# chubbymaggie/syzkaller

Hardware: AMD Instinct MI355X
Metric: signal elems triaged/sec (Diff+Merge) (higher is better)
Workload: dtype u32

## Files before the change

syzkaller_amd/csrc/agg.hip:

```cpp
#include <algorithm>
#include <vector>

#include "decide.h"
#include "internal.h"

namespace syz {

constexpr uint32_t kAggThreads = 1024;
constexpr uint32_t kAggSlots = 7424;
constexpr uint32_t kAggBW = 4;
using KBucket = uint4;
constexpr uint32_t kAggBuckets = kAggSlots / kAggBW;
constexpr uint32_t kAggNoSlot = 0xFFFFFFFFu;
static_assert(kAggRegion == kAggSlots, "distinct-list region per partition (internal.h)");
constexpr uint32_t kAggLimit = kAggSlots * 4 / 5;
constexpr double kAggTargetLoad = 0.4;
constexpr double kAggTargetLoadEntry = 0.6;
constexpr uint64_t kMinItems = 2048;
constexpr uint32_t kAggEmpty = 0xFFFFFFFFu;
constexpr uint32_t kAggOverflow = 0xFFFFFFFFu;
constexpr uint32_t kAggMinBits = 3, kAggMaxBits = 11;
constexpr uint32_t kAggMaxParts = 1u << kAggMaxBits;
constexpr uint32_t kAggTile = 18432;
constexpr uint32_t kAggGroup = 8;
constexpr uint32_t kAggU = 4, kAggD = 2;

struct AggGeom {
	uint32_t pbits;
	uint32_t ibits;
	__host__ __device__ uint32_t rbits() const { return 32 - pbits; }
	__host__ __device__ uint32_t cbits() const { return pbits - 2; }
	__host__ __device__ uint32_t items_per_chunk_log2() const { return cbits() - ibits; }
	__host__ __device__ uint32_t part(uint32_t h) const { return h >> (32 - pbits); }
	__host__ __device__ uint32_t meta(uint32_t level, uint64_t serial) const
	{
		return (level << cbits()) | ((uint32_t)serial & ((1u << cbits()) - 1));
	}
	__host__ __device__ uint32_t rec(uint32_t h, uint32_t meta) const { return (h << pbits) | meta; }
	__host__ __device__ uint32_t resid(uint32_t r) const { return r >> pbits; }
	__host__ __device__ uint32_t level(uint32_t r) const { return (r >> cbits()) & 3; }
	__host__ __device__ uint32_t local(uint32_t r) const { return r & ((1u << cbits()) - 1); }
};

__device__ __forceinline__ uint32_t agg_home_bucket(uint32_t key, const AggGeom& g)
{
	return __umulhi(key << g.pbits, kAggBuckets);
}

__device__ __forceinline__ uint32_t lds_flag(uint32_t* f)
{
	return __hip_atomic_load(f, __ATOMIC_RELAXED, __HIP_MEMORY_SCOPE_WORKGROUP);
}
__device__ __forceinline__ void lds_flag_set(uint32_t* f)
{
	__hip_atomic_store(f, 1u, __ATOMIC_RELAXED, __HIP_MEMORY_SCOPE_WORKGROUP);
}

__device__ __forceinline__ uint32_t bucket_find(uint4 B, uint32_t e)
{
	return B.x == e ? 0 : B.y == e ? 1 : B.z == e ? 2 : B.w == e ? 3 : 4;
}

__device__ __forceinline__ uint32_t bucket_first_empty(uint4 B)
{
	return B.x == kAggEmpty ? 0 : B.y == kAggEmpty ? 1 : B.z == kAggEmpty ? 2 : B.w == kAggEmpty ? 3 : 4;
}

__device__ uint32_t agg_find_insert(KBucket* kb, uint32_t e, uint32_t b, KBucket B, uint32_t* s_ovf, uint32_t& ins)
{
	uint32_t* keys = reinterpret_cast<uint32_t*>(kb);
	for (uint32_t step = 0; step < kAggBuckets;) {
		const uint32_t f = bucket_find(B, e);
		if (f < kAggBW)
			return b * kAggBW + f;
		const uint32_t j = bucket_first_empty(B);
		if (j == kAggBW) {
			b = b + 1 == kAggBuckets ? 0 : b + 1;
			B = kb[b];
			step++;
			continue;
		}
		const uint32_t i = b * kAggBW + j;
		const uint32_t key = atomicCAS(&keys[i], kAggEmpty, e);
		if (key == kAggEmpty) {
			ins++;
			return i;
		}
		if (key == e)
			return i;
		B = kb[b];
	}
	lds_flag_set(s_ovf);
	return kAggNoSlot;
}

struct CellGroup {
	uint64_t ch0;
	uint32_t bnd[kAggGroup + 1];
	__device__ void load(const uint32_t* __restrict__ ot, uint64_t nchunks, uint64_t gi)
	{
		ch0 = gi * kAggGroup;
#pragma unroll
		for (uint32_t i = 0; i <= kAggGroup; i++)
			bnd[i] = ot[min<uint64_t>(ch0 + i, nchunks)];
	}
	__device__ uint32_t serial(uint32_t j, uint32_t r, const AggGeom& g) const
	{
		uint32_t chunk = (uint32_t)ch0;
#pragma unroll
		for (uint32_t i = 1; i < kAggGroup; i++)
			chunk += j >= bnd[i];
		return (chunk << g.cbits()) | g.local(r);
	}
};

template <bool kShard>
__global__ __launch_bounds__(kAggThreads) void k_agg_count(const uint32_t* __restrict__ sigs,
                                                           const uint64_t* __restrict__ call_start,
                                                           const uint32_t* __restrict__ call_len, uint64_t c0,
                                                           uint64_t c1, AggGeom g, AggSrc x, uint32_t* counts)
{
	__shared__ uint32_t h[kAggMaxParts];
	auto add = [&](uint32_t e) {
		if (!kShard || owner_of(e, x.nshards) == x.shard)
			atomicAdd(&h[g.part(fmix32(e))], 1u);
	};
	const uint32_t P = 1u << g.pbits, cb = g.ibits;
	const uint32_t w = threadIdx.x >> 6, nw = blockDim.x >> 6, lane = lane_id();
	const uint64_t ncalls = c1 - c0, nchunks = (ncalls + (1ull << cb) - 1) >> cb;
	for (uint64_t ch = blockIdx.x; ch < nchunks; ch += gridDim.x) {
		for (uint32_t i = threadIdx.x; i < P; i += blockDim.x)
			h[i] = 0;
		__syncthreads();
		const uint64_t ce = min<uint64_t>(ncalls, (ch + 1) << cb);
		for (uint64_t s = (ch << cb) + w; s < ce; s += nw) {
			const uint64_t c = c0 + s, start = call_start[c];
			const uint32_t len = call_len[c];
			uint32_t j = lane;
			for (; j + 192 < len; j += 256) {
				const uint32_t a = sigs[start + j], b = sigs[start + j + 64], d = sigs[start + j + 128],
				               f = sigs[start + j + 192];
				add(a);
				add(b);
				add(d);
				add(f);
			}
			for (; j < len; j += 64)
				add(sigs[start + j]);
		}
		__syncthreads();
		for (uint32_t i = threadIdx.x; i < P; i += blockDim.x)
			counts[ch * P + i] = h[i];
		__syncthreads();
	}
}

__device__ __forceinline__ uint32_t block_excl_scan_1k(uint32_t v, uint32_t* out)
{
	__shared__ uint32_t wsum[16];
	const uint32_t lane = lane_id(), w = threadIdx.x >> 6, nw = blockDim.x >> 6;
	uint32_t x = v;
#pragma unroll
	for (int o = 1; o < 64; o <<= 1) {
		const uint32_t y = __shfl_up(x, o, 64);
		if (lane >= (uint32_t)o)
			x += y;
	}
	if (lane == 63)
		wsum[w] = x;
	__syncthreads();
	uint32_t pre = 0, tot = 0;
	for (uint32_t i = 0; i < nw; i++) {
		pre += i < w ? wsum[i] : 0;
		tot += wsum[i];
	}
	__syncthreads();
	*out = pre + x - v;
	return tot;
}

__global__ __launch_bounds__(1024) void k_agg_scan_chunks(const uint32_t* counts, uint64_t nitems, uint32_t ilog,
                                                          uint32_t P, uint32_t* offs, uint32_t* offsT, uint64_t* totals)
{
	const uint32_t p = blockIdx.x;
	const uint64_t nchunks = (nitems + (1ull << ilog) - 1) >> ilog;
	uint32_t* ot = offsT + (uint64_t)p * (nchunks + 1);
	uint64_t run = 0;
	for (uint64_t b0 = 0; b0 < nitems; b0 += blockDim.x) {
		const uint64_t b = b0 + threadIdx.x;
		const uint32_t v = b < nitems ? counts[b * P + p] : 0;
		uint32_t ex;
		const uint32_t tot = block_excl_scan_1k(v, &ex);
		if (b < nitems) {
			offs[b * P + p] = (uint32_t)(run + ex);
			if ((b & ((1ull << ilog) - 1)) == 0)
				ot[b >> ilog] = (uint32_t)(run + ex);
		}
		run += tot;
	}
	if (threadIdx.x == 0) {
		totals[p] = run;
		ot[nchunks] = (uint32_t)run;
	}
}

__global__ __launch_bounds__(1024) void k_agg_scan_totals(const uint64_t* totals, uint32_t P, uint64_t* rec_base)
{
	__shared__ uint64_t wsum[16];
	const uint32_t lane = lane_id(), w = threadIdx.x >> 6, i0 = threadIdx.x * 2;
	const uint64_t a = i0 < P ? totals[i0] : 0, b = i0 + 1 < P ? totals[i0 + 1] : 0;
	uint64_t x = a + b;
#pragma unroll
	for (int o = 1; o < 64; o <<= 1) {
		const uint64_t y = __shfl_up(x, o, 64);
		if (lane >= (uint32_t)o)
			x += y;
	}
	if (lane == 63)
		wsum[w] = x;
	__syncthreads();
	uint64_t pre = 0, tot = 0;
	for (uint32_t k = 0; k < 16; k++) {
		pre += k < w ? wsum[k] : 0;
		tot += wsum[k];
	}
	const uint64_t ex = pre + x - (a + b);
	if (i0 < P)
		rec_base[i0] = ex;
	if (i0 + 1 < P)
		rec_base[i0 + 1] = ex + a;
	if (threadIdx.x == 0)
		rec_base[P] = tot;
}

constexpr uint32_t kScatChunkMax = 1u << (kAggMaxBits - 2);
constexpr uint32_t kScatWaves = kAggThreads / 64;

constexpr uint32_t kScat3K = 16;
constexpr uint32_t kScat3KEntry = 10;
constexpr uint32_t kScat3Fill = 85;
constexpr uint32_t kScatPer = 12;
constexpr uint32_t kScatPerEntry = 10;
constexpr uint32_t kBlk = 16;
constexpr uint32_t kDummyLines = 2048;
typedef uint32_t scat_v4u __attribute__((ext_vector_type(4)));

struct CapCells {
	const uint64_t* base;
	const uint32_t* cap;
	uint32_t* cnt;
	uint32_t* ovf;
	uint64_t nchunks;
	uint32_t* dummy;
	const uint64_t* sizes = nullptr;
	const uint32_t* tiles = nullptr;
	bool split = false;
	uint32_t tile = 1024;
};

constexpr uint32_t kScat3Tile = kScat3K * 64, kScat3TileEntry = kScat3KEntry * 64;
__host__ __device__ inline uint64_t scat3_tiles(uint32_t len, uint32_t tile)
{
	return (len + tile - 1) / tile;
}
__device__ inline bool scat3_takes(uint64_t recs, uint32_t tiles, uint32_t tile)
{
	return recs * 100 >= (uint64_t)tiles * tile * kScat3Fill;
}

template <bool kOn>
struct PrioLevels {
	uint8_t lvl[kOn ? 256 : 1];
	__device__ __forceinline__ void load(const LevelMap& lm, uint32_t nthreads)
	{
		if (kOn) {
			for (uint32_t i = threadIdx.x; i < 256; i += nthreads)
				lvl[i] = lm.lvl[i];
		}
	}
	__device__ __forceinline__ uint32_t level(uint32_t pv, bool kept, bool& bad) const
	{
		const uint32_t lv = lvl[kOn ? pv : 0];
		bad |= kept && lv == 0xff;
		return lv & 3;
	}
	static __device__ __forceinline__ void report(bool bad, const AggSrc& x)
	{
		if (kOn && x.bad_level && __ballot(bad) && lane_id() == 0)
			atomicOr(x.bad_level, 1u);
	}
};

struct CallTable {
	uint64_t start[kScatChunkMax];
	uint32_t len[kScatChunkMax];
	uint16_t meta[kScatChunkMax];
	template <bool kEntry>
	__device__ __forceinline__ void load(const uint64_t* __restrict__ call_start, const uint32_t* __restrict__ call_len,
	                                     const uint8_t* __restrict__ call_prio, const LevelMap& lm, const AggGeom& g,
	                                     uint64_t c0, uint64_t cbeg, uint32_t nc)
	{
		for (uint32_t i = threadIdx.x; i < nc; i += blockDim.x) {
			const uint64_t c = c0 + cbeg + i;
			start[i] = call_start[c];
			len[i] = call_len[c];
			meta[i] = (uint16_t)g.meta(kEntry ? 0 : lm.lvl[call_prio[c]], cbeg + i);
		}
	}
	__device__ __forceinline__ uint32_t call_of(uint32_t w, uint32_t loc) const { return w + (loc >> 24) * kScatWaves; }
	template <bool kEntry, uint32_t kPer>
	__device__ __forceinline__ uint32_t fetch(uint32_t w, uint32_t lane, uint32_t nc, uint32_t& wc, uint32_t& wo,
	                                          const uint32_t* __restrict__ sigs, const AggSrc& x, uint32_t (&ev)[kPer],
	                                          uint32_t (&loc)[kPer], uint32_t (&pv)[kEntry ? kPer : 1]) const
	{
		constexpr uint32_t kQuota = kPer * 64;
		uint32_t q = 0;
		while (q < kQuota && wc < nc) {
			const uint32_t ln = len[wc], m = min(kQuota - q, ln - wo);
			const uint32_t tag = ((wc - w) / kScatWaves) << 24;
			if (q == 0) {
#pragma unroll
				for (uint32_t u = 0; u < kPer; u++)
					loc[u] = tag | wo;
			}
#pragma unroll
			for (uint32_t u = 0; u < kPer; u++) {
				const uint32_t i = u * 64 + lane;
				loc[u] = i >= q && i < q + m ? tag | (wo + i - q) : loc[u];
			}
			q += m;
			wo += m;
			if (wo == ln) {
				wc += kScatWaves;
				wo = 0;
			}
		}
		if (q) {
#pragma unroll
			for (uint32_t u = 0; u < kPer; u++) {
				const uint64_t a = start[call_of(w, loc[u])] + (loc[u] & 0xFFFFFFu);
				ev[u] = __builtin_nontemporal_load(&sigs[a]);
				if (kEntry)
					pv[kEntry ? u : 0] = (uint8_t)__builtin_nontemporal_load(&x.elem_prio[a]);
			}
		}
		return q;
	}
};

template <bool kEntry>
__global__ __launch_bounds__(kAggThreads) void k_agg_scatter(const uint32_t* __restrict__ sigs,
                                                             const uint64_t* __restrict__ call_start,
                                                             const uint32_t* __restrict__ call_len,
                                                             const uint8_t* __restrict__ call_prio, LevelMap lm,
                                                             uint64_t c0, uint64_t c1, AggGeom g, AggSrc x,
                                                             const uint32_t* __restrict__ offs,
                                                             const uint64_t* __restrict__ rec_base, uint32_t* recs)
{
	constexpr uint32_t kQuota = kAggTile / kScatWaves, kPer = kQuota / 64;
	static_assert(kQuota % 64 == 0, "tile quota per wave");
	__shared__ uint32_t t_rec[kAggTile];
	__shared__ uint16_t t_part[kAggTile];
	__shared__ uint64_t cur[kAggMaxParts];
	__shared__ uint32_t hist[kAggMaxParts], pos[kAggMaxParts];
	__shared__ CallTable calls;
	__shared__ PrioLevels<kEntry> levels;
	const uint32_t P = 1u << g.pbits, cb = g.cbits(), ib = g.ibits;
	levels.load(lm, blockDim.x);
	const uint32_t w = threadIdx.x >> 6, lane = lane_id();
	const uint64_t ncalls = c1 - c0, nitems = (ncalls + (1ull << ib) - 1) >> ib;
	const uint32_t per_t = (P + blockDim.x - 1) / blockDim.x;
	bool badlv = false;
	for (uint64_t ch = blockIdx.x; ch < nitems; ch += gridDim.x) {
		const uint64_t cbeg = ch << ib;
		const uint32_t nc = (uint32_t)min<uint64_t>(ncalls - cbeg, 1ull << ib);
		for (uint32_t i = threadIdx.x; i < P; i += blockDim.x) {
			cur[i] = rec_base[i] + offs[ch * P + i];
			hist[i] = 0;
		}
		calls.load<kEntry>(call_start, call_len, call_prio, lm, g, c0, cbeg, nc);
		__syncthreads();
		uint32_t wc = w, wo = 0;
		uint32_t ev[kPer], loc[kPer], pv[kEntry ? kPer : 1];
		auto fetch = [&]() { return calls.fetch<kEntry>(w, lane, nc, wc, wo, sigs, x, ev, loc, pv); };
		uint32_t n = fetch();
		for (;;) {
#pragma unroll
			for (uint32_t u = 0; u < kPer; u++) {
				const uint32_t i = u * 64 + lane;
				const bool keep = i < n && (!kEntry || x.nshards == 1 || owner_of(ev[u], x.nshards) == x.shard);
				if (keep) {
					const uint32_t h = fmix32(ev[u]), p = g.part(h);
					const uint32_t r = atomicAdd(&hist[p], 1u);
					uint32_t meta = calls.meta[calls.call_of(w, loc[u])];
					if (kEntry)
						meta |= levels.level(pv[kEntry ? u : 0], true, badlv) << cb;
					ev[u] = g.rec(h, meta);
					loc[u] = p | (r << 16);
				} else {
					loc[u] = ~0u;
				}
			}
			__syncthreads();
			uint32_t hsum = 0;
			for (uint32_t q = 0; q < per_t; q++) {
				const uint32_t i = threadIdx.x * per_t + q;
				hsum += i < P ? hist[i] : 0;
			}
			uint32_t ex;
			const uint32_t nt = block_excl_scan_1k(hsum, &ex);
			for (uint32_t q = 0; q < per_t; q++) {
				const uint32_t i = threadIdx.x * per_t + q;
				if (i < P) {
					pos[i] = ex;
					cur[i] -= ex;
					ex += hist[i];
				}
			}
			__syncthreads();
#pragma unroll
			for (uint32_t u = 0; u < kPer; u++) {
				if (loc[u] != ~0u) {
					const uint32_t p = loc[u] & 0xFFFFu, d = pos[p] + (loc[u] >> 16);
					t_rec[d] = ev[u];
					t_part[d] = (uint16_t)p;
				}
			}
			n = fetch();
			__syncthreads();
			for (uint32_t d = threadIdx.x; d < nt; d += blockDim.x)
				recs[cur[t_part[d]] + d] = t_rec[d];
			__syncthreads();
			for (uint32_t i = threadIdx.x; i < P; i += blockDim.x) {
				cur[i] += pos[i] + hist[i];
				hist[i] = 0;
			}
			if (!__syncthreads_or(n != 0))
				break;
		}
	}
	PrioLevels<kEntry>::report(badlv, x);
}

struct ScatLane {
	uint32_t w, lane;
	uint32_t seq = 0;
	bool spilled = false;
};
struct ScatItem {
	uint32_t* recs;
	uint64_t base;
	uint32_t cap;
};
template <uint32_t kB>
struct ScatBlocks {
	static_assert(kB == 16 || kB == 32, "block of 64 or 128 B");
	static constexpr uint32_t kMaxP = kB == 16 ? 2048 : 1024;
	static_assert(kMaxP * kB * 4 == 128 * 1024 && kMaxP <= kAggMaxParts, "128 KB of blocks");
	static constexpr uint32_t kG = 64 / kB;
	static constexpr uint32_t kLB = kB / 4, kGF = 64 / kLB;
	static constexpr uint32_t kShare = (kMaxP + kAggThreads - 1) / kAggThreads;
	alignas(16) uint32_t buf[kMaxP * kB];
	uint32_t fillc[kMaxP + 1];
	uint32_t written[kMaxP + 1];
	uint16_t flist[kShare * kAggThreads];
	uint32_t s_or[2][kScatWaves];

	__device__ __forceinline__ void reset(uint32_t P)
	{
		for (uint32_t i = threadIdx.x; i < P; i += kAggThreads) {
			fillc[i] = 0;
			written[i] = 0;
		}
	}
	__device__ __forceinline__ bool wg_or(ScatLane& t, bool pred)
	{
		uint32_t* r = s_or[t.seq++ & 1];
		const bool any = __ballot(pred) != 0;
		if (t.lane == 0)
			r[t.w] = any;
		__syncthreads();
		return __ballot(r[t.lane & (kScatWaves - 1)] != 0) != 0;
	}
	template <uint32_t M>
	__device__ __forceinline__ uint32_t place(const uint32_t (&rec)[M], const uint32_t (&pt)[M], uint32_t pend)
	{
		uint32_t sl[M];
#pragma unroll
		for (uint32_t u = 0; u < M; u++)
			sl[u] = (pend >> u) & 1 ? atomicAdd(&fillc[pt[u]], 1u) : kB;
#pragma unroll
		for (uint32_t u = 0; u < M; u++) {
			if (sl[u] < kB) {
				buf[pt[u] * kB + sl[u]] = rec[u];
				pend &= ~(1u << u);
			}
		}
		return pend;
	}
	__device__ __forceinline__ void flush(ScatLane& t, uint32_t P, const ScatItem& it, uint32_t* dummy)
	{
		const uint32_t fgrp = t.lane / kLB, fq = t.lane % kLB;
		uint16_t* wl = flist + t.w * kShare * 64;
		uint32_t nw = 0;
#pragma unroll
		for (uint32_t i = 0; i < kShare; i++) {
			const uint32_t p = i * kAggThreads + t.w * 64 + t.lane;
			const bool f = p < P && fillc[p] >= kB;
			const uint64_t m = __ballot(f);
			if (f)
				wl[nw + lane_rank(m)] = (uint16_t)p;
			nw += (uint32_t)__popcll(m);
		}
		for (uint32_t jb = 0; jb < nw; jb += kGF) {
			const bool ok = jb + fgrp < nw;
			const uint32_t pp = wl[min(jb + fgrp, nw - 1)];
			const uint32_t wr = written[pp];
			const scat_v4u v = *reinterpret_cast<const scat_v4u*>(&buf[pp * kB + fq * 4]);
			const bool fits = wr + kB <= it.cap;
			t.spilled |= ok && !fits;
			uint32_t* d = ok && fits ? it.recs + it.base + (uint64_t)pp * it.cap + wr
			                         : dummy + (blockIdx.x % (kDummyLines * kBlk / kB)) * kB;
			*reinterpret_cast<scat_v4u*>(d + fq * 4) = v;
			__builtin_amdgcn_wave_barrier();
			if (fq == 0 && ok) {
				written[pp] = wr + kB;
				fillc[pp] = 0;
			}
		}
	}
	template <uint32_t M>
	__device__ __forceinline__ void scatter_tile(ScatLane& t, uint32_t P, const ScatItem& it, uint32_t* dummy,
	                                             const uint32_t (&rec)[M], const uint32_t (&pt)[M], uint32_t pend)
	{
		for (;;) {
			pend = place(rec, pt, pend);
			const bool more = wg_or(t, pend != 0);
			flush(t, P, it, dummy);
			if (!more)
				break;
			__syncthreads();
		}
	}
	__device__ __forceinline__ void finish(ScatLane& t, uint32_t P, const ScatItem& it, const CapCells& cc, uint64_t ch)
	{
		const uint32_t grp = t.lane / kB, slot = t.lane & (kB - 1);
		for (uint32_t p = t.w * kG + grp; p < P; p += kScatWaves * kG) {
			const uint32_t c = fillc[p], wr = written[p];
			if (wr + c > it.cap)
				t.spilled = true;
			else if (slot < c)
				it.recs[it.base + (uint64_t)p * it.cap + wr + slot] = buf[p * kB + slot];
			if (slot == 0)
				cc.cnt[(uint64_t)p * cc.nchunks + ch] = min(wr + c, it.cap);
		}
		if (t.spilled)
			*cc.ovf = 1u;
		__syncthreads();
	}
};

template <bool kEntry, uint32_t kB>
__global__ __launch_bounds__(kAggThreads, 4) void k_agg_scatter_blk(const uint32_t* __restrict__ sigs,
                                                                    const uint64_t* __restrict__ call_start,
                                                                    const uint32_t* __restrict__ call_len,
                                                                    const uint8_t* __restrict__ call_prio, LevelMap lm,
                                                                    uint64_t c0, uint64_t c1, AggGeom g, AggSrc x,
                                                                    CapCells cc, uint32_t* recs)
{
	constexpr uint32_t kPer = kEntry ? kScatPerEntry : kScatPer;
	__shared__ ScatBlocks<kB> blocks;
	__shared__ CallTable calls;
	__shared__ PrioLevels<kEntry> levels;
	const uint32_t P = 1u << g.pbits, cb = g.cbits(), ib = g.ibits;
	ScatLane t{threadIdx.x >> 6, lane_id()};
	const uint32_t w = t.w, lane = t.lane;
	const uint64_t ncalls = c1 - c0, nchunks = (ncalls + (1ull << ib) - 1) >> ib;
	if (*cc.ovf)
		return;
	bool badlv = false;
	levels.load(lm, blockDim.x);
	for (uint64_t ch = blockIdx.x; ch < nchunks; ch += gridDim.x) {
		const uint64_t cbeg = ch << ib;
		const uint32_t nc = (uint32_t)min<uint64_t>(ncalls - cbeg, 1ull << ib);
		if (cc.split && scat3_takes(cc.sizes[ch], cc.tiles[ch], cc.tile))
			continue;
		const ScatItem it{recs, cc.base[ch], cc.cap[ch]};
		blocks.reset(P);
		calls.load<kEntry>(call_start, call_len, call_prio, lm, g, c0, cbeg, nc);
		__syncthreads();
		uint32_t wc = w, wo = 0;
		uint32_t ev[kPer], loc[kPer], pv[kEntry ? kPer : 1];
		uint32_t n = calls.fetch<kEntry>(w, lane, nc, wc, wo, sigs, x, ev, loc, pv);
		for (;;) {
			uint32_t rec[kPer], pt[kPer], pend = 0;
#pragma unroll
			for (uint32_t u = 0; u < kPer; u++) {
				const uint32_t h = fmix32(ev[u]);
				pt[u] = g.part(h);
				uint32_t meta = calls.meta[calls.call_of(w, loc[u])];
				const bool keep = !kEntry || x.nshards == 1 || owner_of(ev[u], x.nshards) == x.shard;
				if (kEntry)
					meta |= levels.level(pv[kEntry ? u : 0], u * 64 + lane < n && keep, badlv) << cb;
				rec[u] = g.rec(h, meta);
				pend |= (uint32_t)(u * 64 + lane < n && keep) << u;
			}
			n = calls.fetch<kEntry>(w, lane, nc, wc, wo, sigs, x, ev, loc, pv);
			blocks.scatter_tile(t, P, it, cc.dummy, rec, pt, pend);
			if (!blocks.wg_or(t, n != 0))
				break;
		}
		blocks.finish(t, P, it, cc, ch);
	}
	PrioLevels<kEntry>::report(badlv, x);
}

template <uint32_t kK, bool kEntry, uint32_t kB>
__global__ __launch_bounds__(kAggThreads, 4) void k_scat3(const uint32_t* __restrict__ sigs,
                                                          const uint64_t* __restrict__ call_start,
                                                          const uint32_t* __restrict__ call_len,
                                                          const uint8_t* __restrict__ call_prio, LevelMap lm,
                                                          uint64_t c0, uint64_t c1, AggGeom g, CapCells cc,
                                                          uint32_t* recs, AggSrc x)
{
	constexpr uint32_t kTile = kK * 64;
	static_assert(kK <= 31, "pending masks are 32-bit");
	__shared__ ScatBlocks<kB> blocks;
	__shared__ PrioLevels<true> levels;
	const uint32_t P = 1u << g.pbits;
	ScatLane t{(uint32_t)__builtin_amdgcn_readfirstlane(threadIdx.x >> 6), lane_id()};
	const uint32_t w = t.w, lane = t.lane;
	const uint64_t ncalls = c1 - c0, nchunks = (ncalls + (1ull << g.ibits) - 1) >> g.ibits;
	if (*cc.ovf)
		return;
	bool badlv = false;
	levels.load(lm, kAggThreads);
	for (uint64_t ch = blockIdx.x; ch < nchunks; ch += gridDim.x) {
		const uint64_t cbeg = ch << g.ibits;
		const uint32_t nc = (uint32_t)min<uint64_t>(ncalls - cbeg, 1ull << g.ibits);
		if (cc.split && !scat3_takes(cc.sizes[ch], cc.tiles[ch], cc.tile))
			continue;
		const ScatItem it{recs, cc.base[ch], cc.cap[ch]};
		blocks.reset(P);
		__syncthreads();
		uint32_t j = w, wo = 0, clen = 0, cmeta = 0;
		uint64_t cstart = 0;
		auto open_call = [&]() {
			while (j < nc) {
				const uint64_t c = c0 + cbeg + j;
				clen = call_len[c];
				if (clen) {
					cstart = call_start[c];
					const uintptr_t pa = (uintptr_t)(call_prio + c);
					const uint32_t word =
					    *(const __attribute__((address_space(4))) uint32_t*)(pa & ~(uintptr_t)3);
					cmeta = g.meta(kEntry ? 0 : levels.lvl[(word >> (8 * (pa & 3))) & 0xFF], cbeg + j);
					return;
				}
				j += kScatWaves;
			}
		};
		open_call();
		auto fetch = [&](uint32_t (&v)[kK], uint32_t (&pv)[kEntry ? kK : 1], uint32_t& n, uint32_t& meta) {
			n = j < nc ? min(kTile, clen - wo) : 0u;
			meta = cmeta;
			const uint32_t* src = sigs + cstart + wo;
			const uint32_t last = n ? n - 1 : 0;
#pragma unroll
			for (uint32_t u = 0; u < kK; u++)
				v[u] = __builtin_nontemporal_load(&src[min(u * 64 + lane, last)]);
			if constexpr (kEntry) {
				const int8_t* psrc = x.elem_prio + cstart + wo;
#pragma unroll
				for (uint32_t u = 0; u < kK; u++)
					pv[u] = (uint8_t)__builtin_nontemporal_load(&psrc[min(u * 64 + lane, last)]);
			}
			if (n) {
				wo += n;
				if (wo == clen) {
					wo = 0;
					j += kScatWaves;
					open_call();
				}
			}
		};
		auto tile = [&](const uint32_t (&v)[kK], const uint32_t (&pv)[kEntry ? kK : 1], uint32_t n, uint32_t meta) {
			uint32_t rec[kK], pt[kK];
#pragma unroll
			for (uint32_t u = 0; u < kK; u++) {
				const uint32_t h = fmix32(v[u]);
				pt[u] = g.part(h);
				uint32_t m = meta;
				if constexpr (kEntry)
					m |= levels.level(pv[kEntry ? u : 0], u * 64 + lane < n, badlv) << g.cbits();
				rec[u] = g.rec(h, m);
			}
			const uint32_t nu = n > lane ? (n - lane + 63) >> 6 : 0u;
			blocks.scatter_tile(t, P, it, cc.dummy, rec, pt, (1u << nu) - 1);
		};
		uint32_t va[kK], vb[kK], pa[kEntry ? kK : 1], pb[kEntry ? kK : 1], na, nb, ma, mb;
		fetch(va, pa, na, ma);
		for (;;) {
			fetch(vb, pb, nb, mb);
			tile(va, pa, na, ma);
			if (!blocks.wg_or(t, nb != 0))
				break;
			fetch(va, pa, na, ma);
			tile(vb, pb, nb, mb);
			if (!blocks.wg_or(t, na != 0))
				break;
		}
		blocks.finish(t, P, it, cc, ch);
	}
	PrioLevels<kEntry>::report(badlv, x);
}

static uint64_t nchunks_of(uint64_t ncalls, uint32_t ibits)
{
	return (ncalls + (1ull << ibits) - 1) >> ibits;
}

static void launch_capped_scatter(hipStream_t s, const syzsig_batch* b, uint64_t c0, uint64_t c1, const LevelMap& lm,
                                  const AggGeom& g, CapCells cc, uint32_t* recs, const AggSrc* xp)
{
	const uint32_t grid = (uint32_t)std::min<uint64_t>(cc.nchunks, 2048);
	const bool wide = g.pbits < kAggMaxBits;
	const AggSrc x = xp ? *xp : AggSrc{nullptr, 1, 0, 0};
	auto launch = [&](auto kernel, auto... tail) {
		kernel<<<grid, kAggThreads, 0, s>>>(b->sigs, b->call_start, b->call_len, b->call_prio, lm, c0, c1, g, tail...);
	};
	if (!xp || xp->nshards == 1) {
		cc.split = xp || (cc.sizes && cc.tiles);
		if (!xp)
			launch(k_scat3<kScat3K, false, 16>, cc, recs, x);
		else if (wide)
			launch(k_scat3<kScat3KEntry, true, 32>, cc, recs, x);
		else
			launch(k_scat3<kScat3KEntry, true, 16>, cc, recs, x);
		if (!cc.split)
			return;
	}
	if (xp)
		launch(wide ? k_agg_scatter_blk<true, 32> : k_agg_scatter_blk<true, 16>, x, cc, recs);
	else
		launch(wide ? k_agg_scatter_blk<false, 32> : k_agg_scatter_blk<false, 16>, x, cc, recs);
}

__global__ __launch_bounds__(256) void k_chunk_sizes(const uint32_t* __restrict__ call_len, uint64_t c0, uint64_t c1,
                                                     uint32_t cbits, uint64_t* sizes, uint32_t* tiles, uint32_t tile)
{
	const uint64_t ch = blockIdx.x, cbeg = c0 + (ch << cbits), cend = min<uint64_t>(c1, cbeg + (1ull << cbits));
	uint64_t s = 0, t = 0;
	for (uint64_t c = cbeg + threadIdx.x; c < cend; c += blockDim.x) {
		s += call_len[c];
		t += scat3_tiles(call_len[c], tile);
	}
	s = wave_sum_u64(s);
	t = wave_sum_u64(t);
	__shared__ uint64_t ws[4][2];
	if (lane_id() == 0) {
		ws[threadIdx.x >> 6][0] = s;
		ws[threadIdx.x >> 6][1] = t;
	}
	__syncthreads();
	if (threadIdx.x == 0) {
		sizes[ch] = ws[0][0] + ws[1][0] + ws[2][0] + ws[3][0];
		if (tiles)
			tiles[ch] = (uint32_t)min<uint64_t>(ws[0][1] + ws[1][1] + ws[2][1] + ws[3][1], 0xFFFFFFFFu);
	}
}

__device__ __forceinline__ void cell_plan(const uint64_t* __restrict__ sizes, uint64_t nchunks, uint32_t P, float sd,
                                          uint64_t* base, uint32_t* cap)
{
	__shared__ uint64_t wsum[16];
	uint64_t run = 0;
	for (uint64_t b0 = 0; b0 < nchunks; b0 += blockDim.x) {
		const uint64_t c = b0 + threadIdx.x;
		uint64_t v = 0;
		if (c < nchunks) {
			const float m = (float)sizes[c] / (float)P;
			const uint32_t k = sd < 0 ? 64u : ((uint32_t)(m + sd * sqrtf(m)) + 64 + 63) & ~63u;
			cap[c] = k;
			v = (uint64_t)k * P;
		}
		uint64_t xs = v;
		const uint32_t lane = lane_id(), w = threadIdx.x >> 6;
#pragma unroll
		for (int o = 1; o < 64; o <<= 1) {
			const uint64_t y = __shfl_up(xs, o, 64);
			if (lane >= (uint32_t)o)
				xs += y;
		}
		if (lane == 63)
			wsum[w] = xs;
		__syncthreads();
		uint64_t pre = 0, tot = 0;
		for (uint32_t i = 0; i < 16; i++) {
			pre += i < w ? wsum[i] : 0;
			tot += wsum[i];
		}
		if (c < nchunks)
			base[c] = run + pre + xs - v;
		run += tot;
		__syncthreads();
	}
}

__global__ __launch_bounds__(1024) void k_cell_plan(const uint64_t* __restrict__ sizes, uint64_t nchunks, uint32_t P,
                                                    float sd, uint64_t* base, uint32_t* cap)
{
	cell_plan(sizes, nchunks, P, sd, base, cap);
}

__global__ __launch_bounds__(256) void k_fast_prep(const uint64_t* __restrict__ call_start,
                                                   const uint32_t* __restrict__ call_len,
                                                   const uint8_t* __restrict__ call_prio, uint64_t c0, uint64_t c1,
                                                   uint32_t ibits, uint64_t nrec_space, uint64_t* sizes,
                                                   uint64_t* part, uint8_t* call_new, LevelMap lm, uint32_t* tiles)
{
	const uint64_t ch = blockIdx.x, cbeg = c0 + (ch << ibits), cend = min<uint64_t>(c1, cbeg + (1ull << ibits));
	uint64_t tot = 0, bad = 0, other = 0, nt = 0;
	for (uint64_t c = cbeg + threadIdx.x; c < cend; c += blockDim.x) {
		const uint64_t st = call_start[c];
		const uint32_t ln = call_len[c];
		tot += ln;
		nt += scat3_tiles(ln, kScat3Tile);
		bad += st > nrec_space || ln > nrec_space - st || ln > kSerialMask;
		other |= lm.lvl[call_prio[c]] == 0xff;
		call_new[c] = 0;
	}
	tot = wave_sum_u64(tot);
	bad = wave_sum_u64(bad);
	other = wave_sum_u64(other);
	nt = wave_sum_u64(nt);
	__shared__ uint64_t ws[4][4];
	if (lane_id() == 0) {
		ws[threadIdx.x >> 6][0] = tot;
		ws[threadIdx.x >> 6][1] = bad;
		ws[threadIdx.x >> 6][2] = other;
		ws[threadIdx.x >> 6][3] = nt;
	}
	__syncthreads();
	if (threadIdx.x == 0) {
		uint64_t t = 0, b = 0, o = 0, tl = 0;
		for (int w = 0; w < 4; w++) {
			t += ws[w][0];
			b += ws[w][1];
			o += ws[w][2];
			tl += ws[w][3];
		}
		sizes[ch] = t;
		if (tiles)
			tiles[ch] = (uint32_t)min<uint64_t>(tl, 0xFFFFFFFFu);
		part[2 * ch] = t;
		part[2 * ch + 1] = b | (o ? 1ull << 63 : 0);
	}
}

__global__ __launch_bounds__(1024) void k_cell_plan_fast(const uint64_t* __restrict__ sizes, uint64_t nchunks,
                                                         uint32_t P, float sd, uint64_t* base, uint32_t* cap,
                                                         const uint64_t* __restrict__ part, uint64_t guess,
                                                         uint64_t npairs0, unsigned long long* ctr)
{
	__shared__ unsigned long long s_tot, s_flag;
	if (threadIdx.x == 0) {
		s_tot = 0;
		s_flag = 0;
	}
	if (threadIdx.x < kNumCounters)
		ctr[threadIdx.x] = threadIdx.x == kCntAux2 ? npairs0 : 0;
	__syncthreads();
	uint64_t t = 0, f = 0;
	for (uint64_t c = threadIdx.x; c < nchunks; c += blockDim.x) {
		t += part[2 * c];
		f |= part[2 * c + 1];
	}
	t = wave_sum_u64(t);
	for (int o = 32; o > 0; o >>= 1)
		f |= __shfl_xor(f, o, 64);
	if (lane_id() == 0) {
		atomicAdd(&s_tot, (unsigned long long)t);
		atomicOr(&s_flag, (unsigned long long)f);
	}
	__syncthreads();
	if (threadIdx.x == 0) {
		ctr[kCntRecords] = s_tot;
		ctr[kCntSpill] = (s_flag >> 63 ? 2u : 0u) | ((s_flag & ~(1ull << 63)) || s_tot > guess ? 4u : 0u);
	}
	cell_plan(sizes, nchunks, P, sd, base, cap);
}

struct AggLds {
	KBucket kb[kAggBuckets];
	uint32_t fl[4][kAggSlots];
	uint2 q[kAggThreads / 64][64];
	uint32_t s_n, s_ovf, s_out, s_next;
};

struct AggCells {
	const uint32_t* recs;
	const uint64_t* rec_base;
	const uint32_t* offsT;
	const uint64_t* cap_base;
	const uint32_t* cap_len;
	const uint32_t* cap_cnt;
	uint64_t nchunks;
	uint32_t ilog, gsz;
	const uint32_t* spill;
	unsigned long long* ctr;
};

template <uint32_t U, uint32_t D, bool kCap, bool kIdx32>
__device__ __forceinline__ bool agg_partition(AggLds& L, uint32_t p, const AggCells& x, const AggGeom& g)
{
	KBucket* kb = L.kb;
	auto& fl = L.fl;
	const uint32_t* __restrict__ recs = x.recs;
	const uint64_t* __restrict__ rec_base = x.rec_base;
	const uint32_t* __restrict__ offsT = x.offsT;
	const uint64_t* __restrict__ cap_base = x.cap_base;
	const uint32_t* __restrict__ cap_len = x.cap_len;
	const uint32_t* __restrict__ cap_cnt = x.cap_cnt;
	const uint64_t nchunks = x.nchunks;
	const uint32_t ilog = x.ilog, gsz = x.gsz;
	const uint32_t lane = lane_id();
	uint2* wq = L.q[threadIdx.x >> 6];
	uint32_t qn = 0;
	auto flush_queue = [&]() {
		uint32_t ins = 0;
		if (lds_flag(&L.s_ovf)) {
			qn = 0;
			return;
		}
		if (lane < qn) {
			const uint2 e = wq[lane];
			const uint32_t hb = __umulhi(e.x << g.pbits, kAggBuckets);
			const uint32_t slot = agg_find_insert(kb, e.x, hb, kb[hb], &L.s_ovf, ins);
			if (slot != kAggNoSlot)
				atomicMin(&fl[e.y >> 24][slot], e.y & 0xFFFFFFu);
		}
		const uint32_t n_ins = (uint32_t)wave_sum_u64(ins);
		if (n_ins && lane == 0 && atomicAdd(&L.s_n, n_ins) + n_ins > kAggLimit)
			lds_flag_set(&L.s_ovf);
		qn = 0;
		__builtin_amdgcn_wave_barrier();
	};
	const uint64_t ngroups = (nchunks + gsz - 1) / gsz;
	for (uint32_t i = threadIdx.x; i < kAggSlots; i += blockDim.x) {
		if (i < kAggSlots)
			reinterpret_cast<uint32_t*>(kb)[i] = kAggEmpty;
		fl[0][i] = fl[1][i] = fl[2][i] = fl[3][i] = kNoFirst;
	}
	if (threadIdx.x == 0) {
		L.s_n = 0;
		L.s_ovf = 0;
		L.s_out = 0;
		L.s_next = 0;
	}
	__syncthreads();
	const uint32_t* ot = offsT + (uint64_t)p * (nchunks + 1);
	for (;;) {
		uint32_t gi = 0;
		if (lane == 0)
			gi = atomicAdd(&L.s_next, 1u);
		gi = __builtin_amdgcn_readfirstlane(__shfl(gi, 0, 64));
		if (gi >= ngroups || lds_flag(&L.s_ovf))
			break;
		const uint64_t ch0 = (uint64_t)gi * gsz;
		uint64_t lbase = 0;
		uint32_t llen = 0;
		{
			const uint64_t c = ch0 + lane;
			if (lane < gsz && c < nchunks) {
				if (kCap) {
					lbase = cap_base[c] + (uint64_t)p * cap_len[c];
					llen = cap_cnt[(uint64_t)p * nchunks + c];
				} else {
					lbase = rec_base[p] + ot[c];
					llen = ot[c + 1] - ot[c];
				}
			}
		}
		uint32_t lvs = llen;
#pragma unroll
		for (uint32_t o = 1; o < 64; o <<= 1) {
			if (o < gsz) {
				const uint32_t y = __shfl_up(lvs, o, 64);
				if (lane >= o)
					lvs += y;
			}
		}
		const uint32_t n = __builtin_amdgcn_readlane(lvs, gsz - 1);
		if (n == 0)
			continue;
		lvs -= llen;
		const uint64_t ldelta = lbase - lvs;
		const uint32_t nl = n - 1;
		auto cells = [&](uint32_t o0, uint32_t& c0, uint64_t& inside) {
			c0 = (uint32_t)__popcll(__ballot(lane < gsz && lvs <= o0)) - 1;
			inside = __ballot(lane < gsz && lvs > o0 && lvs < o0 + U * 64);
		};
		auto delta_of = [&](uint32_t i) -> uint64_t {
			const uint32_t lo = __builtin_amdgcn_readlane((uint32_t)ldelta, i);
			const uint32_t hi = __builtin_amdgcn_readlane((uint32_t)(ldelta >> 32), i);
			return (uint64_t)hi << 32 | lo;
		};
		auto fetch = [&](uint32_t (&buf)[U], uint32_t o0) {
			uint32_t c0;
			uint64_t inside;
			cells(min(o0, nl), c0, inside);
			if constexpr (kIdx32) {
				const uint32_t d0 = __builtin_amdgcn_readlane((uint32_t)ldelta, c0);
				uint32_t v[U], d[U];
#pragma unroll
				for (uint32_t u = 0; u < U; u++) {
					v[u] = min(o0 + u * 64 + lane, nl);
					d[u] = d0;
				}
				for (uint64_t m = inside; m; m &= m - 1) {
					const uint32_t j = __builtin_ctzll(m), vs = __builtin_amdgcn_readlane(lvs, j);
					const uint32_t dj = __builtin_amdgcn_readlane((uint32_t)ldelta, j);
#pragma unroll
					for (uint32_t u = 0; u < U; u++)
						d[u] = v[u] >= vs ? dj : d[u];
				}
#pragma unroll
				for (uint32_t u = 0; u < U; u++)
					buf[u] = __builtin_nontemporal_load(&recs[v[u] + d[u]]);
				return;
			}
			const uint64_t d0 = delta_of(c0);
			uint32_t v[U];
			uint64_t d[U];
#pragma unroll
			for (uint32_t u = 0; u < U; u++) {
				v[u] = min(o0 + u * 64 + lane, nl);
				d[u] = d0;
			}
			for (uint64_t m = inside; m; m &= m - 1) {
				const uint32_t j = __builtin_ctzll(m), vs = __builtin_amdgcn_readlane(lvs, j);
				const uint64_t dj = delta_of(j);
#pragma unroll
				for (uint32_t u = 0; u < U; u++)
					d[u] = v[u] >= vs ? dj : d[u];
			}
#pragma unroll
			for (uint32_t u = 0; u < U; u++)
				buf[u] = __builtin_nontemporal_load(&recs[v[u] + d[u]]);
		};
		auto absorb = [&](const uint32_t (&buf)[U], uint32_t o0) {
			uint32_t c0;
			uint64_t inside;
			cells(o0, c0, inside);
			uint32_t key[U], lv[U], k[U], hb[U], slot[U], c[U];
#pragma unroll
			for (uint32_t u = 0; u < U; u++)
				c[u] = (uint32_t)ch0 + c0;
			for (uint64_t m = inside; m; m &= m - 1) {
				const uint32_t vs = __builtin_amdgcn_readlane(lvs, __builtin_ctzll(m));
#pragma unroll
				for (uint32_t u = 0; u < U; u++)
					c[u] += min(o0 + u * 64 + lane, nl) >= vs;
			}
#pragma unroll
			for (uint32_t u = 0; u < U; u++) {
				const uint32_t r = buf[u];
				k[u] = ((c[u] >> ilog) << g.cbits()) | g.local(r);
				key[u] = g.resid(r);
				lv[u] = g.level(r);
				hb[u] = __umulhi(r & ~((1u << g.pbits) - 1), kAggBuckets);
			}
			KBucket B[U];
#pragma unroll
			for (uint32_t u = 0; u < U; u++)
				B[u] = kb[hb[u]];
			bool any_need = false;
#pragma unroll
			for (uint32_t u = 0; u < U; u++) {
				const uint32_t f = bucket_find(B[u], key[u]);
				slot[u] = f < kAggBW ? hb[u] * kAggBW + f : kAggNoSlot;
				any_need |= f >= kAggBW;
			}
			if (__builtin_amdgcn_readfirstlane((uint32_t)(__ballot(any_need) != 0))) {
#pragma unroll
				for (uint32_t u = 0; u < U; u++) {
					const bool nd = slot[u] == kAggNoSlot;
					const uint64_t m = __ballot(nd);
					if (!m)
						continue;
					const uint32_t c = (uint32_t)__popcll(m);
					if (qn + c > 64)
						flush_queue();
					if (nd)
						wq[qn + lane_rank(m)] = make_uint2(key[u], (lv[u] << 24) | k[u]);
					qn += c;
				}
				__builtin_amdgcn_wave_barrier();
			}
#pragma unroll
			for (uint32_t u = 0; u < U; u++)
				if (slot[u] != kAggNoSlot)
					atomicMin(&fl[lv[u]][slot[u]], k[u]);
		};
		uint32_t buf[D + 1][U];
#pragma unroll
		for (uint32_t d = 0; d < D; d++)
			fetch(buf[d], d * U * 64);
		bool more = true;
		for (uint32_t o0 = 0; more;) {
#pragma unroll
			for (uint32_t t = 0; t <= D; t++) {
				if (more) {
					fetch(buf[(t + D) % (D + 1)], o0 + D * U * 64);
					absorb(buf[t], o0);
					o0 += U * 64;
					more = o0 < n;
				}
			}
		}
	}
	flush_queue();
	__syncthreads();
	return !L.s_ovf;
}

template <uint32_t U, uint32_t D, bool kCap, bool kIdx32 = false>
__global__ __launch_bounds__(kAggThreads) void k_agg(AggCells x, AggGeom g, uint32_t* dist_e, uint4* dist_f,
                                                     uint32_t* cnt)
{
	__shared__ AggLds L;
	const uint32_t* keys = reinterpret_cast<const uint32_t*>(L.kb);
	const uint32_t P = 1u << g.pbits, lane = lane_id();
	if (x.spill && *x.spill)
		return;
	for (uint32_t p = blockIdx.x; p < P; p += gridDim.x) {
		if (!agg_partition<U, D, kCap, kIdx32>(L, p, x, g)) {
			if (threadIdx.x == 0) {
				cnt[p] = kAggOverflow;
				if (x.ctr)
					atomicAdd(&x.ctr[kCntAggOvf], 1ull);
			}
			__syncthreads();
			continue;
		}
		const uint32_t hp = p << g.rbits();
		for (uint32_t i0 = 0; i0 < kAggSlots; i0 += kAggThreads) {
			const uint32_t i = i0 + threadIdx.x;
			const uint32_t key = i < kAggSlots ? keys[i] : kAggEmpty;
			const bool occ = key != kAggEmpty;
			const uint64_t m = __ballot(occ);
			uint32_t wb = 0;
			if (lane == 0 && m)
				wb = atomicAdd(&L.s_out, (uint32_t)__popcll(m));
			wb = __shfl(wb, 0, 64);
			if (occ) {
				const uint64_t o = (uint64_t)p * kAggRegion + wb + lane_rank(m);
				dist_e[o] = fmix32_inv(hp | key);
				dist_f[o] = make_uint4(L.fl[0][i], L.fl[1][i], L.fl[2][i], L.fl[3][i]);
			}
		}
		__syncthreads();
		if (threadIdx.x == 0) {
			cnt[p] = L.s_out;
			if (x.ctr && L.s_out)
				atomicAdd(&x.ctr[kCntDistinct], (unsigned long long)L.s_out);
		}
		__syncthreads();
	}
}

template <bool kCap>
static void launch_agg(const syzsig_ctx* ctx, uint64_t extent, uint32_t P, hipStream_t s, const AggCells& xc,
                       const AggGeom& g, void* de, void* df, void* dc)
{
	if (extent <= (1ull << 32) && !(ctx->agg_dbg & SYZSIG_DEBUG_AGG_IDX64))
		k_agg<kAggU, kAggD, kCap, true><<<P, kAggThreads, 0, s>>>(xc, g, (uint32_t*)de, (uint4*)df, (uint32_t*)dc);
	else
		k_agg<kAggU, kAggD, kCap, false><<<P, kAggThreads, 0, s>>>(xc, g, (uint32_t*)de, (uint4*)df, (uint32_t*)dc);
}

__device__ __forceinline__ void hbm_absorb(uint32_t* gkeys, uint32_t* gfl, uint64_t C, uint32_t h, uint32_t level,
                                           uint32_t serial, uint64_t& bad)
{
	uint64_t i = C;
	if (h != kAggEmpty) {
		i = fmix32(h ^ 0x632BE5ABu) & (C - 1);
		for (uint64_t step = 0;; step++) {
			uint32_t key = gkeys[i];
			if (key == kAggEmpty) {
				key = atomicCAS(&gkeys[i], kAggEmpty, h);
				if (key == kAggEmpty)
					break;
			}
			if (key == h)
				break;
			i = (i + 1) & (C - 1);
			if (step >= C) {
				bad++;
				return;
			}
		}
	}
	atomicMin(&gfl[(uint64_t)level * (C + 1) + i], serial);
}

__global__ __launch_bounds__(256) void k_agg_global(const uint32_t* __restrict__ recs,
                                                    const uint64_t* __restrict__ rec_base,
                                                    const uint32_t* __restrict__ offsT, uint64_t nchunks, AggGeom g,
                                                    const uint32_t* __restrict__ ovl, uint32_t novl, uint32_t* gkeys,
                                                    uint32_t* gfl, uint64_t C, unsigned long long* err)
{
	const uint32_t lane = lane_id();
	const uint64_t ngroups = (nchunks + kAggGroup - 1) / kAggGroup, items = (uint64_t)novl * ngroups;
	const uint64_t nwaves = (uint64_t)gridDim.x * (blockDim.x >> 6);
	uint64_t bad = 0;
	for (uint64_t it = blockIdx.x * (uint64_t)(blockDim.x >> 6) + (threadIdx.x >> 6); it < items; it += nwaves) {
		const uint32_t p = ovl[it / ngroups];
		const uint32_t* ot = offsT + (uint64_t)p * (nchunks + 1);
		const uint32_t* pr = recs + rec_base[p];
		CellGroup cg;
		cg.load(ot, nchunks, it % ngroups);
		for (uint32_t j = cg.bnd[0] + lane; j < cg.bnd[kAggGroup]; j += 64) {
			const uint32_t r = pr[j];
			const uint32_t k = cg.serial(j, r, g), l = g.level(r);
			const uint32_t h = (p << g.rbits()) | g.resid(r);
			hbm_absorb(gkeys, gfl, C, h, l, k, bad);
		}
	}
	block_count(err, bad);
}

__global__ __launch_bounds__(256) void k_agg_global_compact(const uint32_t* __restrict__ gkeys,
                                                            const uint32_t* __restrict__ gfl, uint64_t C,
                                                            uint32_t* dist_e, uint4* dist_f,
                                                            unsigned long long* out_cnt)
{
	const uint32_t lane = lane_id();
	for (uint64_t i0 = blockIdx.x * (uint64_t)blockDim.x; i0 <= C; i0 += (uint64_t)gridDim.x * blockDim.x) {
		const uint64_t i = i0 + threadIdx.x;
		bool occ = false;
		uint32_t h = kAggEmpty;
		uint4 f = make_uint4(kNoFirst, kNoFirst, kNoFirst, kNoFirst);
		if (i <= C) {
			f = make_uint4(gfl[i], gfl[(C + 1) + i], gfl[2 * (C + 1) + i], gfl[3 * (C + 1) + i]);
			if (i < C) {
				h = gkeys[i];
				occ = h != kAggEmpty;
			} else {
				occ = (f.x & f.y & f.z & f.w) != kNoFirst;
			}
		}
		const uint64_t m = __ballot(occ);
		unsigned long long wb = 0;
		if (lane == 0 && m)
			wb = atomicAdd(out_cnt, (unsigned long long)__popcll(m));
		wb = __shfl(wb, 0, 64);
		if (occ) {
			dist_e[wb + lane_rank(m)] = fmix32_inv(h);
			dist_f[wb + lane_rank(m)] = f;
		}
	}
}

struct FinArgs {
	LevelMap lm;
	uint64_t c0;
	uint64_t* slots;
	uint64_t bmask;
	uint64_t* ns_slots;
	uint64_t ns_bmask;
	uint8_t* call_new;
	uint64_t* pairs;
	unsigned long long* npairs;
	unsigned long long* ctr;
	uint32_t ms_shift, ns_shift;
	uint32_t* def_e;
	uint4* def_f;
	unsigned long long* def_cnt;
	uint64_t* def_ns;
	unsigned long long* def_ns_cnt;
	uint32_t dbg;
	const uint32_t* spill;
	const unsigned long long* ovf_gate;
	uint32_t gate_max;
};

template <typename Put>
__device__ __forceinline__ void fin_emit(const FinArgs& a, uint32_t e, uint4 f4, int top, int p0, Put put)
{
	stair_walk(f4, top, [&](int l) { return (int)a.lm.val[l] <= p0; },
	           [&](int, uint32_t first) {
		           const uint64_t c = a.c0 + first;
		           a.call_new[c] = 1;
		           put((c << 32) | e);
	           });
}

__device__ __forceinline__ bool fin_commit_atomic(const FinArgs& a, uint32_t e, int8_t P, FinCounts& n, int& p0,
                                                  const Bucket* bm = nullptr, const Bucket* bn = nullptr)
{
	const uint64_t word = make_slot(e, P), max_probe = max_probe_for(a.bmask);
	uint64_t old = 0;
	const int64_t idx = bm ? tbl_find_or_insert_from(a.slots, a.bmask, e, word, old, max_probe, *bm)
	                       : tbl_find_or_insert(a.slots, a.bmask, e, word, old, max_probe);
	if (idx < 0) {
		n.ovf++;
		return false;
	}
	if (!fin_raises(old, P, n, p0))
		return false;
	if (old != 0)
		a.slots[idx] = word;
	const int rr = bn ? tbl_merge_from(a.ns_slots, a.ns_bmask, e, P, *bn) : tbl_merge(a.ns_slots, a.ns_bmask, e, P);
	n.ns_ins += rr == 1;
	n.ovf += rr < 0;
	return true;
}

template <uint32_t kCap>
struct PairBuf {
	uint64_t buf[kCap];
	uint32_t n;
	unsigned long long base;
	__device__ __forceinline__ void reset()
	{
		if (threadIdx.x == 0)
			n = 0;
	}
	__device__ __forceinline__ void emit(uint64_t v, uint64_t* pairs, unsigned long long* npairs)
	{
		const uint32_t k = atomicAdd(&n, 1u);
		if (k < kCap)
			buf[k] = v;
		else
			pairs[atomicAdd(npairs, 1ull)] = v;
	}
	__device__ __forceinline__ void flush_if_half(uint64_t* pairs, unsigned long long* npairs)
	{
		__syncthreads();
		const uint32_t nb = n;
		if (nb > kCap / 2)
			flush(nb, pairs, npairs);
	}
	__device__ __forceinline__ void flush_all(uint64_t* pairs, unsigned long long* npairs)
	{
		__syncthreads();
		const uint32_t nb = n;
		if (nb)
			flush(nb, pairs, npairs);
	}
	__device__ __forceinline__ void flush(uint32_t nb, uint64_t* pairs, unsigned long long* npairs)
	{
		nb = min(nb, kCap);
		if (threadIdx.x == 0)
			base = atomicAdd(npairs, (unsigned long long)nb);
		__syncthreads();
		for (uint32_t t = threadIdx.x; t < nb; t += blockDim.x)
			pairs[base + t] = buf[t];
		__syncthreads();
		reset();
		__syncthreads();
	}
};

template <uint32_t kIlp, uint32_t kThreads>
struct FinElems {
	uint32_t e[kIlp];
	uint4 f4[kIlp];
	int top[kIlp];
	__device__ __forceinline__ void load(const uint32_t* __restrict__ dist_e, const uint4* __restrict__ dist_f,
	                                     uint32_t r, uint32_t n, uint32_t i0, const LevelMap& lm)
	{
#pragma unroll
		for (uint32_t k = 0; k < kIlp; k++) {
			const uint32_t i = i0 + k * kThreads + threadIdx.x;
			const uint64_t o = (uint64_t)r * kAggRegion + min(i, n - 1);
			e[k] = dist_e[o];
			f4[k] = dist_f[o];
			top[k] = fin_top(f4[k], lm, i < n);
		}
	}
};

constexpr uint32_t kFinThreads = 256, kFinBuf = 4 * kFinThreads * 2, kFinIlp = 2;

__global__ __launch_bounds__(kFinThreads) void k_agg_finalize(const uint32_t* __restrict__ dist_e,
                                                              const uint4* __restrict__ dist_f,
                                                              const uint32_t* __restrict__ cnt, uint32_t nregions,
                                                              FinArgs a)
{
	__shared__ PairBuf<kFinBuf> pb;
	FinCounts n;
	const auto put = [&](uint64_t v) { pb.emit(v, a.pairs, a.npairs); };
	pb.reset();
	__syncthreads();
	for (uint32_t r = blockIdx.x; r < nregions; r += gridDim.x) {
		const uint32_t nr = cnt[r] == kAggOverflow ? 0 : cnt[r];
		for (uint32_t i0 = 0; i0 < nr; i0 += kFinIlp * kFinThreads) {
			FinElems<kFinIlp, kFinThreads> t;
			t.load(dist_e, dist_f, r, nr, i0, a.lm);
			Bucket bm[kFinIlp], bn[kFinIlp];
#pragma unroll
			for (uint32_t k = 0; k < kFinIlp; k++) {
				if (t.top[k] >= 0) {
					bm[k] = load_bucket(a.slots + (home_bucket(t.e[k], a.bmask) << kBucketShift));
					bn[k] = load_bucket(a.ns_slots + (home_bucket(t.e[k], a.ns_bmask) << kBucketShift));
				}
// ... 1266 lines not shown
```

Measured before the change: 278.4 billion.

## Pad capped cells to quads and fetch records as 128-bit vector loads

```diff
diff --git a/syzkaller_amd/csrc/agg.hip b/syzkaller_amd/csrc/agg.hip
--- a/syzkaller_amd/csrc/agg.hip
+++ b/syzkaller_amd/csrc/agg.hip
@@ -1,4 +1,5 @@
 #include <algorithm>
+#include <type_traits>
 #include <vector>
 
 #include "decide.h"
@@ -243,6 +244,8 @@
 constexpr uint32_t kScatPerEntry = 10;
 constexpr uint32_t kBlk = 16;
 constexpr uint32_t kDummyLines = 2048;
+constexpr uint32_t kCellQuad = 4;
+constexpr uint32_t kCellCapUnit = 64;
 typedef uint32_t scat_v4u __attribute__((ext_vector_type(4)));
 
 struct CapCells {
@@ -544,15 +547,17 @@
 	}
 	__device__ __forceinline__ void finish(ScatLane& t, uint32_t P, const ScatItem& it, const CapCells& cc, uint64_t ch)
 	{
+		static_assert(kB % kCellQuad == 0 && kCellCapUnit % kCellQuad == 0, "blocks and cells are whole quads");
 		const uint32_t grp = t.lane / kB, slot = t.lane & (kB - 1);
 		for (uint32_t p = t.w * kG + grp; p < P; p += kScatWaves * kG) {
 			const uint32_t c = fillc[p], wr = written[p];
+			const uint32_t cq = (c + kCellQuad - 1) & ~(kCellQuad - 1);
 			if (wr + c > it.cap)
 				t.spilled = true;
-			else if (slot < c)
-				it.recs[it.base + (uint64_t)p * it.cap + wr + slot] = buf[p * kB + slot];
+			else if (slot < cq)
+				it.recs[it.base + (uint64_t)p * it.cap + wr + slot] = buf[p * kB + min(slot, c - 1)];
 			if (slot == 0)
-				cc.cnt[(uint64_t)p * cc.nchunks + ch] = min(wr + c, it.cap);
+				cc.cnt[(uint64_t)p * cc.nchunks + ch] = min(wr + cq, it.cap);
 		}
 		if (t.spilled)
 			*cc.ovf = 1u;
@@ -780,6 +785,7 @@
 		uint64_t v = 0;
 		if (c < nchunks) {
 			const float m = (float)sizes[c] / (float)P;
+			static_assert(kCellCapUnit == 64, "cap = .. + 64 rounded up to 64");
 			const uint32_t k = sd < 0 ? 64u : ((uint32_t)(m + sd * sqrtf(m)) + 64 + 63) & ~63u;
 			cap[c] = k;
 			v = (uint64_t)k * P;
@@ -925,6 +931,13 @@
 	const uint64_t nchunks = x.nchunks;
 	const uint32_t ilog = x.ilog, gsz = x.gsz;
 	const uint32_t lane = lane_id();
+	static_assert(!kCap || U == kCellQuad, "a capped-cell batch is one quad per lane");
+	struct Recs {
+		uint32_t r[U];
+		__device__ __forceinline__ uint32_t operator[](uint32_t u) const { return r[u]; }
+		__device__ __forceinline__ uint32_t& operator[](uint32_t u) { return r[u]; }
+	};
+	using Batch = std::conditional_t<kCap, scat_v4u, Recs>;
 	uint2* wq = L.q[threadIdx.x >> 6];
 	uint32_t qn = 0;
 	auto flush_queue = [&]() {
@@ -1006,10 +1019,31 @@
 			const uint32_t hi = __builtin_amdgcn_readlane((uint32_t)(ldelta >> 32), i);
 			return (uint64_t)hi << 32 | lo;
 		};
-		auto fetch = [&](uint32_t (&buf)[U], uint32_t o0) {
+		auto fetch = [&](Batch& buf, uint32_t o0) {
 			uint32_t c0;
 			uint64_t inside;
 			cells(min(o0, nl), c0, inside);
+			if constexpr (kCap) {
+				const uint32_t v = min(o0 + lane * kCellQuad, n - kCellQuad);
+				if constexpr (kIdx32) {
+					uint32_t d = __builtin_amdgcn_readlane((uint32_t)ldelta, c0);
+					for (uint64_t m = inside; m; m &= m - 1) {
+						const uint32_t j = __builtin_ctzll(m), vs = __builtin_amdgcn_readlane(lvs, j);
+						const uint32_t dj = __builtin_amdgcn_readlane((uint32_t)ldelta, j);
+						d = v >= vs ? dj : d;
+					}
+					buf = __builtin_nontemporal_load(reinterpret_cast<const scat_v4u*>(&recs[v + d]));
+				} else {
+					uint64_t d = delta_of(c0);
+					for (uint64_t m = inside; m; m &= m - 1) {
+						const uint32_t j = __builtin_ctzll(m), vs = __builtin_amdgcn_readlane(lvs, j);
+						const uint64_t dj = delta_of(j);
+						d = v >= vs ? dj : d;
+					}
+					buf = __builtin_nontemporal_load(reinterpret_cast<const scat_v4u*>(&recs[v + d]));
+				}
+				return;
+			}
 			if constexpr (kIdx32) {
 				const uint32_t d0 = __builtin_amdgcn_readlane((uint32_t)ldelta, c0);
 				uint32_t v[U], d[U];
@@ -1049,7 +1083,7 @@
 			for (uint32_t u = 0; u < U; u++)
 				buf[u] = __builtin_nontemporal_load(&recs[v[u] + d[u]]);
 		};
-		auto absorb = [&](const uint32_t (&buf)[U], uint32_t o0) {
+		auto absorb = [&](const Batch& buf, uint32_t o0) {
 			uint32_t c0;
 			uint64_t inside;
 			cells(o0, c0, inside);
@@ -1059,9 +1093,18 @@
 				c[u] = (uint32_t)ch0 + c0;
 			for (uint64_t m = inside; m; m &= m - 1) {
 				const uint32_t vs = __builtin_amdgcn_readlane(lvs, __builtin_ctzll(m));
-#pragma unroll
-				for (uint32_t u = 0; u < U; u++)
-					c[u] += min(o0 + u * 64 + lane, nl) >= vs;
+				if constexpr (kCap) {
+					c[0] += min(o0 + lane * kCellQuad, n - kCellQuad) >= vs;
+				} else {
+#pragma unroll
+					for (uint32_t u = 0; u < U; u++)
+						c[u] += min(o0 + u * 64 + lane, nl) >= vs;
+				}
+			}
+			if constexpr (kCap) {
+#pragma unroll
+				for (uint32_t u = 1; u < U; u++)
+					c[u] = c[0];
 			}
 #pragma unroll
 			for (uint32_t u = 0; u < U; u++) {
@@ -1103,7 +1146,7 @@
 				if (slot[u] != kAggNoSlot)
 					atomicMin(&fl[lv[u]][slot[u]], k[u]);
 		};
-		uint32_t buf[D + 1][U];
+		Batch buf[D + 1];
 #pragma unroll
 		for (uint32_t d = 0; d < D; d++)
 			fetch(buf[d], d * U * 64);
```

Result: faster. 288.4 billion (median of 6 runs) (+3.6%).
